# JeffWang987/MVSTER

Hardware: AMD Instinct MI355X
Metric: depth-maps/sec (DTU 512×640, 5-view, 4-stage) at 1/2/4/8 MI355X (higher is better)
Workload: dtype f32; 1 GPU; DTU mid 512x640, 5 views, 4-stage cascade 8/8/4/4 hyp, B=1 eval, 1 depth map(s) per step per GPU; launch=hipGraph replay, parallelism=replicas x1, depth_maps_in_flight_per_gpu=2

## Files before the change

### mvster_amd/csrc/conv_pers.hip

```cpp
#include "conv_args.hpp"

namespace mvconv {
namespace {


#ifdef MVSTER_TIMELINE
__device__ unsigned long long* g_ptl = nullptr;
#define MV_PTL(k)                                                                                                       \
    do {                                                                                                                \
        __builtin_amdgcn_sched_barrier(0);                                                                              \
        if (g_ptl && lane == 0 && it < 16)                                                                              \
            g_ptl[(((size_t)(blockIdx.y * gridDim.x + blockIdx.x) * 4 + wave) * 16 + it) * 8 + (k)] =                    \
                (k) < 5 ? __builtin_amdgcn_s_memtime() : (k) == 5 ? __builtin_amdgcn_s_getreg(63492)                    \
                                                         : (k) == 6 ? __builtin_amdgcn_s_getreg(63508) : tile;          \
        __builtin_amdgcn_sched_barrier(0);                                                                              \
    } while (0)
#define MV_PPTL(k, v)                                                                                                   \
    do {                                                                                                                \
        __builtin_amdgcn_sched_barrier(0);                                                                              \
        if (g_ptl && lane == 0 && hp < 16)                                                                              \
            g_ptl[(((size_t)(blockIdx.y * gridDim.x + blockIdx.x) * 8 + wave8) * 16 + hp) * 4 + (k)] = (v);           \
        __builtin_amdgcn_sched_barrier(0);                                                                              \
    } while (0)
#else
// ... 572 lines not shown
#pragma unroll
                    for (int c = 0; c < NCH; ++c) {
                        const f32x4v w = wl[(wbase + tap * NCH + c) * 64 + lane];
                        f32x4v A[MT];
#pragma unroll
                        for (int mt = 0; mt < MT; ++mt) A[mt] = patch[abase[mt] + c * 2 * PLANE + cbase + dy * RS + dx * 2];
#pragma unroll
                        for (int j = 0; j < 4; ++j)
#pragma unroll
                            for (int mt = 0; mt < MT; ++mt) acc[mt] = __builtin_amdgcn_mfma_f32_16x16x4f32(w[j], A[mt][j], acc[mt], 0, 0, 0);
                    }
                }
            wbase += kh * kw * NCH;
#pragma unroll
            for (int mt = 0; mt < MT; ++mt) {
                f32x4v v = acc[mt];
#pragma unroll
                for (int j = 0; j < 4; ++j) {
                    v[j] = fmaf(v[j], scv[j], shv[j]);
                    if (a.relu) v[j] = fmaxf(v[j], 0.0f);
                    if (SKIP) v[j] += skv[mt][j];
                }
                __builtin_amdgcn_raw_buffer_store_b128(__builtin_bit_cast(u32x4v, v), out_rsrc, ooff[mt], 0, MV_STORE_AUX);
            }
        }
        __builtin_amdgcn_s_waitcnt(0xc07f);
        __builtin_amdgcn_s_barrier();
    }
}

#ifdef MVSTER_PROBES
template <int MT, int NT, int KW, int SW, int NCH, int KD, bool WREG, int PF, bool SKIP>
__global__ void __launch_bounds__(512) conv_pp_kernel(ConvArgs a, PersArgs p) {
    using G = PersGeom<MT, KW, SW, KD>;
    constexpr int TY = G::TY, KH = G::KH, PW = G::PW, PH = G::PH, PWH = G::PWH, PLANE = G::PLANE, NBLK = G::NBLK;
    constexpr int NTAP = KD * KH * KW, TAPS2D = KH * KW;
    constexpr int BUF = NCH * 2 * PLANE;
    constexpr int NI = NCH * 2 * NBLK;
    constexpr int NIW = (NI + 3) / 4;
    constexpr int CIN = NCH * 16;
    extern __shared__ __attribute__((aligned(16))) float lds_raw[];
    const int lane = threadIdx.x & 63;
    const int wave8 = __builtin_amdgcn_readfirstlane(threadIdx.x >> 6);
    const int grp = wave8 >> 2;
    const int wave = wave8 & 3;
    f32x4v* const lds = reinterpret_cast<f32x4v*>(lds_raw) + grp * 2 * BUF;
    f32x4v* const scratch = reinterpret_cast<f32x4v*>(lds_raw) + 4 * BUF;
    f32x4v* const wl = scratch + 64;
    const int lm = lane & 15, lq = lane >> 4;
    const int nt0 = blockIdx.y * NT;
    const __amdgpu_buffer_rsrc_t in_rsrc =
        __builtin_amdgcn_make_buffer_rsrc(const_cast<float*>(a.in), (short)0, (int)a.in_bytes, 0x00020000);

    unsigned dbase[NIW];
    int dpos[NIW];
#pragma unroll
    for (int n = 0; n < NIW; ++n) {
        const int i = wave + 4 * n;
        const int c = i / (2 * NBLK), r = i - c * 2 * NBLK, pl = r / NBLK, blk = r - pl * NBLK;
        const int s = blk * 64 + lane;
        const int q1 = s & 1;
        int prow, px;
        if (SW == 1) {
            const int pix = s >> 1;
            prow = pix / PW;
            px = pix - prow * PW;
        } else {
            int t = s >> 1;
            const int xh = t % PWH;
            t /= PWH;
            prow = t >> 1;
            px = 2 * xh + (t & 1);
        }
        const bool valid = i < NI && prow < G::ROWS && px < PW;
        const int pz = KD == 1 ? 0 : prow / PH, py = prow - pz * PH;
        dpos[n] = px | (py << 8) | (pz << 16);
        dbase[n] = valid ? (unsigned)(((pz * a.Hi + py) * a.Wi + px) * (CIN * 4) + (c * 16 + pl * 8 + q1 * 4) * 4) : 0x80000000u;
    }

    auto decode_tile = [&](unsigned tile) -> TilePos {
        TilePos t;
        auto div = [&](unsigned n, int k) -> unsigned { return ((__umulhi(n, p.mul[k]) >> p.shr[k]) & ~p.one[k]) | (n & p.one[k]); };
        unsigned q = div(tile, 0);
        t.tx0 = (int)(tile - q * p.tiles_x) * 32;
        unsigned q2 = div(q, 1);
        t.ty0 = (int)(q - q2 * p.tiles_y) * TY;
        const unsigned q3 = div(q2, 2);
        t.zo = (int)(q2 - q3 * (unsigned)a.Do);
        t.b = (int)q3;
        return t;
    };

    auto dma_tile = [&](const TilePos& t, int buf, bool live) {
        const int iz0 = t.zo * a.sd - a.pd[0], iy0 = t.ty0 * SW - a.ph[0], ix0 = t.tx0 * SW - a.pw[0];
        const unsigned origin = (unsigned)((((t.b * a.Di + iz0) * a.Hi + iy0) * a.Wi + ix0) * (CIN * 4));
        const unsigned wi = live ? (unsigned)a.Wi : 0u;
        f32x4v* const dst0 = lds + buf * BUF;
#pragma unroll
        for (int n = 0; n < NIW; ++n) {
            const int i = wave + 4 * n;
            {
                const int ix = ix0 + (dpos[n] & 255), iy = iy0 + ((dpos[n] >> 8) & 255), iz = iz0 + (dpos[n] >> 16);
                bool ok = (unsigned)iy < (unsigned)a.Hi && (unsigned)ix < wi;
                if (KD > 1) ok = ok && (unsigned)iz < (unsigned)a.Di;
                const unsigned off = ok ? dbase[n] + origin : 0x80000000u;
                f32x4v* const dst = (NI % 4 == 0 || n + 1 < NIW || i < NI) ? dst0 + (i / NBLK) * PLANE + (i % NBLK) * 64 : scratch;
                __builtin_amdgcn_raw_ptr_buffer_load_lds(in_rsrc, (lds_void*)dst, 16, off, 0, 0, 0);
            }
        }
    };

    const unsigned nwg = gridDim.x;
    const unsigned first = xcd_remap(blockIdx.x, nwg);
    const unsigned ntl = first < p.ntiles ? (p.ntiles - first + nwg - 1) / nwg : 0u;
    const int kcount = (int)((ntl + 1u - (unsigned)grp) >> 1);
    auto tile_of = [&](int k) -> unsigned { return first + (unsigned)(2 * k + grp) * nwg; };
    if (kcount > 0) dma_tile(decode_tile(tile_of(0)), 0, true);
    if (grp == 0 && kcount > 1) dma_tile(decode_tile(tile_of(1)), 1, true);
    f32x4v wreg[WREG ? NTAP * NCH * NT : 1];
    const long wstep = (long)a.ntile_total * 256;
    if (WREG) {
#pragma unroll
        for (int s = 0; s < NTAP * NCH; ++s)
#pragma unroll
            for (int nt = 0; nt < NT; ++nt)
                wreg[s * NT + nt] = *reinterpret_cast<const f32x4v*>(a.wpk + s * wstep + ((long)(nt0 + nt) * 64 + lane) * 4);
    } else {
        const __amdgpu_buffer_rsrc_t w_rsrc = __builtin_amdgcn_make_buffer_rsrc(
            const_cast<float*>(a.wpk), (short)0, (int)(NTAP * NCH * wstep * 4), 0x00020000);
        for (int i = wave8; i < NTAP * NCH * NT; i += 8) {
            const int s = i / NT, nt = i - s * NT;
            const unsigned off = (unsigned)((s * wstep + (long)(nt0 + nt) * 256) * 4) + lane * 16;
            __builtin_amdgcn_raw_ptr_buffer_load_lds(w_rsrc, (lds_void*)(wl + i * 64), 16, off, 0, 0, 0);
        }
    }
    f32x4v scv[NT], shv[NT];
#pragma unroll
    for (int nt = 0; nt < NT; ++nt) {
        const int n0 = (nt0 + nt) * 16 + lq * 4;
        scv[nt] = *reinterpret_cast<const f32x4v*>(a.scale + n0);
        shv[nt] = *reinterpret_cast<const f32x4v*>(a.shift + n0);
    }
    int abase[MT];
#pragma unroll
    for (int mt = 0; mt < MT; ++mt) {
        const int t = wave * MT + mt;
        const int row = t >> 1, x = (t & 1) * 16 + lm;
        const int rs = G::ROWSLOTS;
        abase[mt] = (SW == 1 ? row * rs + x * 2 : row * 2 * rs + x * 2) + (lq >> 1) * PLANE + (lq & 1);
    }
    const __amdgpu_buffer_rsrc_t out_rsrc =
        __builtin_amdgcn_make_buffer_rsrc(a.out, (short)0, (int)p.out_bytes, 0x00020000);
    const __amdgpu_buffer_rsrc_t skip_rsrc = __builtin_amdgcn_make_buffer_rsrc(
        const_cast<float*>(SKIP ? a.skip : a.in), (short)0, SKIP ? (int)p.out_bytes : 0, 0x00020000);
    unsigned obase[MT];
    int orc[MT];
#pragma unroll
    for (int mt = 0; mt < MT; ++mt) {
        const int t = wave * MT + mt;
        const int row = t >> 1, col = (t & 1) * 16 + lm;
        orc[mt] = row | (col << 8);
        obase[mt] = (unsigned)((row * a.Wo + col) * a.cout + nt0 * 16 + lq * 4) * 4u;
    }
    auto tap_off = [&](int kz, int ky, int kx) -> int {
        const int prow = kz * PH + ky;
        return SW == 1 ? prow * G::ROWSLOTS + kx * 2 : prow * G::ROWSLOTS + (kx & 1) * PWH * 2 + (kx >> 1) * 2;
    };

    __syncthreads();

    f32x4v pacc[MT][NT], pskv[MT][NT];
    unsigned pooff[MT];
#pragma unroll
    for (int mt = 0; mt < MT; ++mt) {
        pooff[mt] = 0x80000000u;
#pragma unroll
        for (int nt = 0; nt < NT; ++nt) pacc[mt][nt] = pskv[mt][nt] = (f32x4v){0.f, 0.f, 0.f, 0.f};
    }
    auto epilogue = [&](const f32x4v (&accv)[MT][NT], const f32x4v (&skvv)[MT][NT], const unsigned (&off)[MT]) {
#pragma unroll
        for (int mt = 0; mt < MT; ++mt) {
#pragma unroll
            for (int nt = 0; nt < NT; ++nt) {
                f32x4v v = accv[mt][nt];
#pragma unroll
                for (int j = 0; j < 4; ++j) {
                    v[j] = fmaf(v[j], scv[nt][j], shv[nt][j]);
                    if (a.relu) v[j] = fmaxf(v[j], 0.0f);
                    if (SKIP) v[j] += skvv[mt][nt][j];
                }
                __builtin_amdgcn_raw_buffer_store_b128(__builtin_bit_cast(u32x4v, v), out_rsrc, off[mt] + nt * 64, 0, MV_STORE_AUX);
            }
        }
    };

    f32x4v skvN[MT][NT];
    unsigned ooffN[MT];
    TilePos here = decode_tile(kcount > 0 ? tile_of(0) : 0u);
#pragma unroll
    for (int mt = 0; mt < MT; ++mt) ooffN[mt] = 0x80000000u;
    const int nhalf = 2 * (int)((ntl + 1u) >> 1) + 1;
    {
        const unsigned oorigin = (unsigned)((((here.b * a.Do + here.zo) * a.Ho + here.ty0) * a.Wo + here.tx0) * a.cout) * 4u;
#pragma unroll
        for (int mt = 0; mt < MT; ++mt) {
            const bool ok = grp == 0 && kcount > 0 && here.ty0 + (orc[mt] & 255) < a.Ho && here.tx0 + (orc[mt] >> 8) < a.Wo;
            ooffN[mt] = ok ? obase[mt] + oorigin : 0x80000000u;
#pragma unroll
            for (int nt = 0; nt < NT; ++nt)
                skvN[mt][nt] = SKIP ? __builtin_bit_cast(f32x4v, __builtin_amdgcn_raw_buffer_load_b128(skip_rsrc, ooffN[mt] + nt * 64, 0, 0))
                                    : (f32x4v){0.f, 0.f, 0.f, 0.f};
        }
    }
    for (int hp = 0; hp < nhalf; ++hp) {
        MV_PPTL(0, __builtin_amdgcn_s_memtime());
        MV_PPTL(3, __builtin_amdgcn_s_getreg(63492));
        if ((hp & 1) == grp) {
            const int k = (hp - grp) >> 1;
            if (k < kcount) {
                const int cur = k & 1;
                f32x4v acc[MT][NT];
#pragma unroll
                for (int mt = 0; mt < MT; ++mt)
#pragma unroll
                    for (int nt = 0; nt < NT; ++nt) acc[mt][nt] = (f32x4v){0.f, 0.f, 0.f, 0.f};
                const f32x4v* patch = lds + cur * BUF;
                const int kz_lo = KD == 1 ? 0 : max(0, a.pd[0] - here.zo * a.sd), kz_hi = KD == 1 ? 1 : min(KD, a.Di + a.pd[0] - here.zo * a.sd);
#pragma unroll
                for (int kz = 0; kz < KD; ++kz) {
                    if (kz < kz_lo || kz >= kz_hi) continue;
                    f32x4v A[PF + 1][NCH][MT], Bv[PF + 1][NCH][NT];
                    auto load_tap = [&](int t2, f32x4v (&Aa)[NCH][MT], f32x4v (&Bb)[NCH][NT]) {
                        const int ky = t2 / KW, kx = t2 - ky * KW;
                        const int to = tap_off(kz, ky, kx);
                        const int tap = kz * TAPS2D + t2;
#pragma unroll
                        for (int c = 0; c < NCH; ++c) {
#pragma unroll
                            for (int mt = 0; mt < MT; ++mt) Aa[c][mt] = patch[abase[mt] + c * 2 * PLANE + to];
#pragma unroll
                            for (int nt = 0; nt < NT; ++nt)
                                Bb[c][nt] = WREG ? wreg[(tap * NCH + c) * NT + nt] : wl[((tap * NCH + c) * NT + nt) * 64 + lane];
                        }
                    };
#pragma unroll
                    for (int t2 = 0; t2 < PF && t2 < TAPS2D; ++t2) load_tap(t2, A[t2 % (PF + 1)], Bv[t2 % (PF + 1)]);
#pragma unroll
                    for (int t2 = 0; t2 < TAPS2D; ++t2) {
                        if (t2 + PF < TAPS2D) load_tap(t2 + PF, A[(t2 + PF) % (PF + 1)], Bv[(t2 + PF) % (PF + 1)]);
#pragma unroll
                        for (int c = 0; c < NCH; ++c)
#pragma unroll
                            for (int j = 0; j < 4; ++j)
#pragma unroll
                                for (int mt = 0; mt < MT; ++mt)
#pragma unroll
                                    for (int nt = 0; nt < NT; ++nt)
                                        acc[mt][nt] = __builtin_amdgcn_mfma_f32_16x16x4f32(Bv[t2 % (PF + 1)][c][nt][j], A[t2 % (PF + 1)][c][mt][j],
                                                                                           acc[mt][nt], 0, 0, 0);
                    }
                }
#pragma unroll
                for (int mt = 0; mt < MT; ++mt) {
                    pooff[mt] = ooffN[mt];
#pragma unroll
                    for (int nt = 0; nt < NT; ++nt) {
                        pacc[mt][nt] = acc[mt][nt];
                        pskv[mt][nt] = skvN[mt][nt];
                    }
                }
            }
            __builtin_amdgcn_s_waitcnt(0xc07f);
            MV_PPTL(2, k < kcount ? 1 : 0);
        } else {
            const int kn = (hp + 1 - grp) >> 1;
            epilogue(pacc, pskv, pooff);
#pragma unroll
            for (int mt = 0; mt < MT; ++mt) pooff[mt] = 0x80000000u;
            __builtin_amdgcn_sched_barrier(0);
            const bool have = kn < kcount;
            here = decode_tile(have ? tile_of(kn) : 0u);
            const unsigned oorigin = (unsigned)((((here.b * a.Do + here.zo) * a.Ho + here.ty0) * a.Wo + here.tx0) * a.cout) * 4u;
#pragma unroll
            for (int mt = 0; mt < MT; ++mt) {
                const bool ok = have && here.ty0 + (orc[mt] & 255) < a.Ho && here.tx0 + (orc[mt] >> 8) < a.Wo;
                ooffN[mt] = ok ? obase[mt] + oorigin : 0x80000000u;
#pragma unroll
                for (int nt = 0; nt < NT; ++nt)
                    skvN[mt][nt] = SKIP ? __builtin_bit_cast(f32x4v, __builtin_amdgcn_raw_buffer_load_b128(skip_rsrc, ooffN[mt] + nt * 64, 0, 0))
                                        : (f32x4v){0.f, 0.f, 0.f, 0.f};
            }
            __builtin_amdgcn_sched_barrier(0);
            const bool more = kn + 1 < kcount;
            dma_tile(decode_tile(more ? tile_of(kn + 1) : 0u), (kn + 1) & 1, more);
            MV_PPTL(2, __builtin_amdgcn_s_memtime());
            asm volatile("s_waitcnt vmcnt(%0)" ::"n"(MT * NT * (SKIP ? 2 : 1) + NIW) : "memory");
        }
        MV_PPTL(1, __builtin_amdgcn_s_memtime());
        __builtin_amdgcn_s_barrier();
    }
}
#endif

template <int NCH, int MT>
__global__ void __launch_bounds__(256) conv1x1_pers_kernel(ConvArgs a, unsigned ngroups, unsigned mtot, unsigned out_bytes) {
    constexpr int CIN = NCH * 16;
    extern __shared__ __attribute__((aligned(16))) float lds_raw[];
    f32x4v* const wl = reinterpret_cast<f32x4v*>(lds_raw);
    const int ntile = a.ntile_total;
    f32x4v* const ssl = wl + NCH * ntile * 64;
    const int lane = threadIdx.x & 63;
    const int wave = __builtin_amdgcn_readfirstlane(threadIdx.x >> 6);
    const int lm = lane & 15, lq = lane >> 4;
    const __amdgpu_buffer_rsrc_t in_rsrc =
        __builtin_amdgcn_make_buffer_rsrc(const_cast<float*>(a.in), (short)0, (int)a.in_bytes, 0x00020000);
    const __amdgpu_buffer_rsrc_t out_rsrc = __builtin_amdgcn_make_buffer_rsrc(a.out, (short)0, (int)out_bytes, 0x00020000);
    const __amdgpu_buffer_rsrc_t skip_rsrc = __builtin_amdgcn_make_buffer_rsrc(
        const_cast<float*>(a.skip_mode ? a.skip : a.in), (short)0,
        a.skip_mode == 1 ? (int)out_bytes : a.skip_mode == 2 ? (int)(out_bytes / 4) : 0, 0x00020000);
    {
        const __amdgpu_buffer_rsrc_t w_rsrc =
            __builtin_amdgcn_make_buffer_rsrc(const_cast<float*>(a.wpk), (short)0, NCH * ntile * 1024, 0x00020000);
        for (int i = wave; i < NCH * ntile; i += 4) {
            const unsigned off = (unsigned)(i * 1024 + lane * 16);
            f32x4v* const dst = wl + i * 64;
            __builtin_amdgcn_raw_ptr_buffer_load_lds(w_rsrc, (lds_void*)dst, 16, off, 0, 0, 0);
        }
        for (int i = threadIdx.x; i < ntile * 4; i += 256) {
            ssl[i] = *reinterpret_cast<const f32x4v*>(a.scale + i * 4);
            ssl[ntile * 4 + i] = *reinterpret_cast<const f32x4v*>(a.shift + i * 4);
        }
    }
    auto load_group = [&](unsigned g, f32x4v (&A)[MT][NCH], unsigned (&vox)[MT]) {
#pragma unroll
        for (int mt = 0; mt < MT; ++mt) {
            const unsigned m = ((g * 4 + wave) * MT + mt) * 16 + lm;
            vox[mt] = m;
#pragma unroll
            for (int c = 0; c < NCH; ++c) {
                const unsigned off = m < mtot ? (m * CIN + c * 16 + lq * 4) * 4u : 0x80000000u;
                A[mt][c] = __builtin_bit_cast(f32x4v, __builtin_amdgcn_raw_buffer_load_b128(in_rsrc, off, 0, 0));
            }
        }
    };
    f32x4v A[MT][NCH], An[MT][NCH];
    unsigned vox[MT], voxn[MT];
    struct Up {
        unsigned o00, o01, o10, o11;
        mv::Lerp ly, lx;
    } up[MT];
    unsigned g = blockIdx.x;
    if (g < ngroups) load_group(g, A, vox);
    __syncthreads();
    const unsigned cout4 = (unsigned)a.cout * 4u;
    for (; g < ngroups; g += gridDim.x) {
        const unsigned gn = g + gridDim.x < ngroups ? g + gridDim.x : g;
        load_group(gn, An, voxn);
        if (a.skip_mode == 2) {
            const int hh = a.HoF / 2, wh = a.WoF / 2;
#pragma unroll
            for (int mt = 0; mt < MT; ++mt) {
                const unsigned m = vox[mt] < mtot ? vox[mt] : 0u;
                const unsigned t = fast_div(m, (unsigned)a.Wo, a.div_mul[0], a.div_shr[0]);
                const int ox = (int)(m - t * (unsigned)a.Wo);
                const unsigned b = fast_div(t, (unsigned)a.Ho, a.div_mul[1], a.div_shr[1]);
                const int oy = (int)(t - b * (unsigned)a.Ho);
                up[mt].ly = mv::make_lerp(oy, hh, a.HoF);
                up[mt].lx = mv::make_lerp(ox, wh, a.WoF);
                const unsigned base = b * (unsigned)(hh * wh);
                up[mt].o00 = (base + up[mt].ly.i0 * wh + up[mt].lx.i0) * cout4;
                up[mt].o01 = (base + up[mt].ly.i0 * wh + up[mt].lx.i1) * cout4;
                up[mt].o10 = (base + up[mt].ly.i1 * wh + up[mt].lx.i0) * cout4;
                up[mt].o11 = (base + up[mt].ly.i1 * wh + up[mt].lx.i1) * cout4;
            }
        }
        f32x4v Bv[NCH];
#pragma unroll
        for (int c = 0; c < NCH; ++c) Bv[c] = wl[(c * ntile) * 64 + lane];
        for (int nt = 0; nt < ntile; ++nt) {
            f32x4v Bn[NCH];
            const int ntn = nt + 1 < ntile ? nt + 1 : nt;
#pragma unroll
            for (int c = 0; c < NCH; ++c) Bn[c] = wl[(c * ntile + ntn) * 64 + lane];
            const f32x4v sc = ssl[nt * 4 + lq], sh = ssl[ntile * 4 + nt * 4 + lq];
            f32x4v acc[MT];
#pragma unroll
            for (int mt = 0; mt < MT; ++mt) acc[mt] = (f32x4v){0.f, 0.f, 0.f, 0.f};
#pragma unroll
            for (int c = 0; c < NCH; ++c)
#pragma unroll
                for (int j = 0; j < 4; ++j)
#pragma unroll
                    for (int mt = 0; mt < MT; ++mt)
                        acc[mt] = __builtin_amdgcn_mfma_f32_16x16x4f32(Bv[c][j], A[mt][c][j], acc[mt], 0, 0, 0);
            const unsigned n0 = (unsigned)(nt * 16 + lq * 4);
#pragma unroll
            for (int mt = 0; mt < MT; ++mt) {
                const unsigned off = (n0 < (unsigned)a.cout && vox[mt] < mtot) ? vox[mt] * cout4 + n0 * 4u : 0x80000000u;
                f32x4v v = acc[mt];
#pragma unroll
                for (int j = 0; j < 4; ++j) {
                    v[j] = fmaf(v[j], sc[j], sh[j]);
                    if (a.relu) v[j] = fmaxf(v[j], 0.0f);
                }
                if (a.skip_mode == 1) {
                    const f32x4v k = __builtin_bit_cast(f32x4v, __builtin_amdgcn_raw_buffer_load_b128(skip_rsrc, off, 0, 0));
#pragma unroll
                    for (int j = 0; j < 4; ++j) v[j] += k[j];
                } else if (a.skip_mode == 2) {
                    const bool ok = n0 < (unsigned)a.cout && vox[mt] < mtot;
                    const unsigned c4 = n0 * 4u;
                    const f32x4v k00 = __builtin_bit_cast(f32x4v, __builtin_amdgcn_raw_buffer_load_b128(skip_rsrc, ok ? up[mt].o00 + c4 : 0x80000000u, 0, 0));
                    const f32x4v k01 = __builtin_bit_cast(f32x4v, __builtin_amdgcn_raw_buffer_load_b128(skip_rsrc, ok ? up[mt].o01 + c4 : 0x80000000u, 0, 0));
                    const f32x4v k10 = __builtin_bit_cast(f32x4v, __builtin_amdgcn_raw_buffer_load_b128(skip_rsrc, ok ? up[mt].o10 + c4 : 0x80000000u, 0, 0));
                    const f32x4v k11 = __builtin_bit_cast(f32x4v, __builtin_amdgcn_raw_buffer_load_b128(skip_rsrc, ok ? up[mt].o11 + c4 : 0x80000000u, 0, 0));
#pragma unroll
                    for (int j = 0; j < 4; ++j) v[j] = mv::bilerp(up[mt].ly, up[mt].lx, k00[j], k01[j], k10[j], k11[j]) + v[j];
                }
                __builtin_amdgcn_raw_buffer_store_b128(__builtin_bit_cast(u32x4v, v), out_rsrc, off, 0, MV_STORE_AUX);
            }
#pragma unroll
            for (int c = 0; c < NCH; ++c) Bv[c] = Bn[c];
        }
#pragma unroll
        for (int mt = 0; mt < MT; ++mt) {
            vox[mt] = voxn[mt];
#pragma unroll
            for (int c = 0; c < NCH; ++c) A[mt][c] = An[mt][c];
        }
    }
}


template <int MT, int NT, int KW, int SW, int NCH, int KD, bool WREG, int PF, bool SKIP, bool LD>
int launch_pers(const ConvArgs& a, int wpc, hipStream_t s) {
    using G = PersGeom<MT, KW, SW, KD>;
    constexpr int NTAP = KD * KW * KW;
    const size_t lds = (size_t)(2 * NCH * 2 * G::PLANE + 64 + (WREG ? 0 : NTAP * NCH * NT * 64)) * 16;
    if (lds > 160 * 1024) return MVSTER_ERR_UNSUPPORTED;
    auto kern = conv_pers_kernel<MT, NT, KW, SW, NCH, KD, WREG, PF, SKIP, LD>;
    static unsigned long attr_done = 0;
    if (lds > 64 * 1024 && !allow_big_lds(reinterpret_cast<const void*>(kern), attr_done)) return MVSTER_ERR_LAUNCH;
    const int g_num_cu = num_cus();
    if (g_num_cu <= 0) return MVSTER_ERR_LAUNCH;
    PersArgs p;
    if (!fill_pers_args(a, G::TY, p)) return MVSTER_ERR_UNSUPPORTED;
    const long ntiles = p.ntiles;
    p.prio = (wpc >> 4) & 1;
    wpc &= 15;
    int by_lds = (int)((160 * 1024) / lds);
    int per_cu = wpc > 0 ? wpc : (by_lds > 3 ? 3 : by_lds);
    if (per_cu > by_lds) per_cu = by_lds;
    if (per_cu < 1) per_cu = 1;
    const int ny = a.ntile_total / NT;
    long gmax = (long)g_num_cu * per_cu / ny;
    if (gmax < 1) gmax = 1;
    const long rounds = (ntiles + gmax - 1) / gmax;
    const long gx = (ntiles + rounds - 1) / rounds;
    MV_NOTE_KERNEL("conv_pers_kernel<%d, %d, %d, %d, %d, %d, %s, %d, %s, %s>", MT, NT, KW, SW, NCH, KD, WREG ? "true" : "false", PF,
                   SKIP ? "true" : "false", LD ? "true" : "false");
    hipLaunchKernelGGL(kern, dim3((unsigned)gx, ny, 1), dim3(LD ? 512 : 256), lds, s, a, p);
    return mv_check_launch();
}

template <int NCH, bool SKIP, int KS>
int launch_tpers(const ConvArgs& a, int wpc, hipStream_t s) {
    using G = PersGeom<2, KS == 5 ? 3 : 2, 1, 1>;
    const size_t lds = (size_t)(2 * NCH * 2 * G::PLANE + 64 + (KS == 5 ? 25 : 9) * NCH * 64) * 16;
    if (lds > 160 * 1024) return MVSTER_ERR_UNSUPPORTED;
    auto kern = conv_tpers_kernel<NCH, SKIP, KS>;
    static unsigned long attr_done = 0;
    if (lds > 64 * 1024 && !allow_big_lds(reinterpret_cast<const void*>(kern), attr_done)) return MVSTER_ERR_LAUNCH;
    const int ncu = num_cus();
    if (ncu <= 0) return MVSTER_ERR_LAUNCH;
    PersArgs p;
    if (!fill_pers_args(a, G::TY, p)) return MVSTER_ERR_UNSUPPORTED;
    const long ntiles = p.ntiles;
    wpc &= 15;
    const int by_lds = (int)((160 * 1024) / lds);
    int per_cu = wpc > 0 ? wpc : 2;
    if (per_cu > by_lds) per_cu = by_lds;
    if (per_cu > 2) per_cu = 2;
    long gmax = (long)ncu * per_cu / a.ntile_total;
    if (gmax < 1) gmax = 1;
    const long rounds = (ntiles + gmax - 1) / gmax;
    const long gx = (ntiles + rounds - 1) / rounds;
    MV_NOTE_KERNEL("conv_tpers_kernel<%d, %s, %d>", NCH, SKIP ? "true" : "false", KS);
    hipLaunchKernelGGL(kern, dim3((unsigned)gx, a.ntile_total, 1), dim3(512), lds, s, a, p);
    return mv_check_launch();
}

template <int KW, bool SKIP>
int launch_pers8(const ConvArgs& a, int wpc, hipStream_t s) {
    using G = PersGeom<2, KW, 2, 1>;
    const size_t lds = (size_t)(2 * G::PLANE + 64) * 16;
    auto kern = conv_pers8_kernel<KW, SKIP>;
    static unsigned long attr_done = 0;
    if (lds > 64 * 1024 && !allow_big_lds(reinterpret_cast<const void*>(kern), attr_done)) return MVSTER_ERR_LAUNCH;
    const int ncu = num_cus();
    if (ncu <= 0) return MVSTER_ERR_LAUNCH;
    PersArgs p;
    if (!fill_pers_args(a, G::TY, p)) return MVSTER_ERR_UNSUPPORTED;
    const long ntiles = p.ntiles;
    wpc &= 15;
    const int by_lds = (int)((160 * 1024) / lds);
    int per_cu = wpc > 0 ? wpc : 2;
    if (per_cu > by_lds) per_cu = by_lds;
    if (per_cu > 3) per_cu = 3;
    const long gmax = (long)ncu * per_cu;
    const long rounds = (ntiles + gmax - 1) / gmax;
    const long gx = (ntiles + rounds - 1) / rounds;
    MV_NOTE_KERNEL("conv_pers8_kernel<%d, %s>", KW, SKIP ? "true" : "false");
    hipLaunchKernelGGL(kern, dim3((unsigned)gx, 1, 1), dim3(512), lds, s, a, p);
    return mv_check_launch();
}

#ifdef MVSTER_PROBES
template <int MT, int NT, int KW, int SW, int NCH, int KD, bool WREG, int PF, bool SKIP>
int launch_pp(const ConvArgs& a, hipStream_t s) {
    using G = PersGeom<MT, KW, SW, KD>;
    constexpr int NTAP = KD * KW * KW;
    const size_t lds = (size_t)(4 * NCH * 2 * G::PLANE + 64 + (WREG ? 0 : NTAP * NCH * NT * 64)) * 16;
    if (lds > 160 * 1024) return MVSTER_ERR_UNSUPPORTED;
    auto kern = conv_pp_kernel<MT, NT, KW, SW, NCH, KD, WREG, PF, SKIP>;
    static unsigned long attr_done = 0;
    if (!allow_big_lds(reinterpret_cast<const void*>(kern), attr_done)) return MVSTER_ERR_LAUNCH;
    const int g_num_cu = num_cus();
    if (g_num_cu <= 0) return MVSTER_ERR_LAUNCH;
    PersArgs p;
    if (!fill_pers_args(a, G::TY, p)) return MVSTER_ERR_UNSUPPORTED;
    const long ntiles = p.ntiles;
    const int ny = a.ntile_total / NT;
    long gmax = (long)g_num_cu / ny;
    if (gmax < 1) gmax = 1;
    long per = (ntiles + gmax - 1) / gmax;
    if (per > 1 && (per & 1)) ++per;
    const long gx = (ntiles + per - 1) / per;
    MV_NOTE_KERNEL("conv_pp_kernel<%d, %d, %d, %d, %d, %d, %s, %d, %s>", MT, NT, KW, SW, NCH, KD, WREG ? "true" : "false", PF,
                   SKIP ? "true" : "false");
    hipLaunchKernelGGL(kern, dim3((unsigned)gx, ny, 1), dim3(512), lds, s, a, p);
    return mv_check_launch();
}
#endif

}

#ifdef MVSTER_TIMELINE
extern "C" int mvster_debug_pers_timeline(void* buf) {
    return hipMemcpyToSymbol(HIP_SYMBOL(g_ptl), &buf, sizeof(buf)) == hipSuccess ? MVSTER_OK : MVSTER_ERR_LAUNCH;
}
#endif

namespace {
template <int NCH, int MT>
int launch_1x1(const ConvArgs& a, int wpc, hipStream_t s) {
    const size_t lds = (size_t)(NCH * a.ntile_total * 64 + 2 * a.ntile_total * 4) * 16;
    const long mtot = (long)a.B * a.Do * a.Ho * a.Wo;
    const long out_bytes = mtot * a.cout * 4;
    if (lds > 160 * 1024 || a.in_bytes >= (1u << 31) || out_bytes >= (1L << 31) || a.cout % 4 != 0) return MVSTER_ERR_UNSUPPORTED;
    auto kern = conv1x1_pers_kernel<NCH, MT>;
    static unsigned long attr_done = 0;
    if (!allow_big_lds(reinterpret_cast<const void*>(kern), attr_done)) return MVSTER_ERR_LAUNCH;
    const int g_num_cu = num_cus();
    if (g_num_cu <= 0) return MVSTER_ERR_LAUNCH;
    const long ngroups = (mtot + 64 * MT - 1) / (64 * MT);
    int by_lds = (int)((160 * 1024) / lds);
    int per_cu = wpc > 0 ? wpc : 2;
    if (per_cu > by_lds) per_cu = by_lds;
    if (per_cu > 4) per_cu = 4;
    const long gmax = (long)g_num_cu * per_cu;
    const long rounds = (ngroups + gmax - 1) / gmax;
    const long gx = (ngroups + rounds - 1) / rounds;
    MV_NOTE_KERNEL("conv1x1_pers_kernel<%d, %d>", NCH, MT);
    hipLaunchKernelGGL(kern, dim3((unsigned)gx), dim3(256), lds, s, a, (unsigned)ngroups, (unsigned)mtot, (unsigned)out_bytes);
    return mv_check_launch();
}
}

int num_cus() {
    static int n = 0;
    if (n == 0) {
        int dev = 0;
        hipDeviceProp_t prop;
        if (hipGetDevice(&dev) != hipSuccess || hipGetDeviceProperties(&prop, dev) != hipSuccess) return 0;
        n = prop.multiProcessorCount;
        if (const char* e = MV_PROBE_ENV("MVSTER_CUS")) {
            const int v = atoi(e);
            if (v > 0 && v <= n) n = v;
        }
    }
    return n;
}

int dispatch_1x1(const ConvArgs& a, int mt, int wpc, hipStream_t s) {
    if (a.nclass != 1 || a.kd[0] != 1 || a.kh[0] != 1 || a.kw[0] != 1 || a.sd != 1 || a.sh != 1 || a.sw != 1 || a.osd != 1 ||
        a.osh != 1 || a.osw != 1 || a.pd[0] != 0 || a.ph[0] != 0 || a.pw[0] != 0 || a.skip_mode > 2 || a.prob_w)
        return MVSTER_ERR_UNSUPPORTED;
    if (a.skip_mode == 2 && (a.Do != 1 || (a.HoF & 1) || (a.WoF & 1))) return MVSTER_ERR_UNSUPPORTED;
    wpc &= 15;
    if (a.cin == 64 && mt == 1) return launch_1x1<4, 1>(a, wpc, s);
    if (a.cin == 64 && mt == 2) return launch_1x1<4, 2>(a, wpc, s);
    if (a.cin == 32 && mt == 1) return launch_1x1<2, 1>(a, wpc, s);
    if (a.cin == 32 && mt == 2) return launch_1x1<2, 2>(a, wpc, s);
    if (a.cin == 32 && mt == 4) return launch_1x1<2, 4>(a, wpc, s);
    if (a.cin == 16 && mt == 2) return launch_1x1<1, 2>(a, wpc, s);
    if (a.cin == 16 && mt == 4) return launch_1x1<1, 4>(a, wpc, s);
    return MVSTER_ERR_UNSUPPORTED;
}

#ifndef MVSTER_PROBES
int dispatch_pp(const ConvArgs&, int, int, hipStream_t) { return MVSTER_ERR_UNSUPPORTED; }
#else
int dispatch_pp(const ConvArgs& a, int mt, int nt, hipStream_t s) {
    if (a.nclass != 1 || a.osd != 1 || a.osh != 1 || a.osw != 1 || a.skip_mode > 1 || a.prob_w || a.cout % 16 != 0 ||
        a.sh != a.sw || a.kh[0] != a.kw[0] || a.ntile_total % nt != 0 || mt != 2 || a.cin % 16 != 0)
        return MVSTER_ERR_UNSUPPORTED;
    const int kd = a.kd[0], kw = a.kw[0], sw = a.sw, nch = a.cin / 16;
#define MV_PP(NT_, KW_, SW_, NCH_, KD_, WREG_, PF_) \
    if (nt == NT_ && kw == KW_ && sw == SW_ && nch == NCH_ && kd == KD_)                                        \
        return a.skip_mode == 1 ? launch_pp<2, NT_, KW_, SW_, NCH_, KD_, WREG_, PF_, true>(a, s)                 \
                                : launch_pp<2, NT_, KW_, SW_, NCH_, KD_, WREG_, PF_, false>(a, s);
    MV_PP(1, 3, 1, 1, 1, true, 2)
    MV_PP(2, 3, 1, 2, 1, false, 1)
    MV_PP(2, 3, 2, 1, 1, true, 1)
#undef MV_PP
    return MVSTER_ERR_UNSUPPORTED;
}
#endif

int dispatch_pers(const ConvArgs& a, int mt, int nt, int wpc, hipStream_t s) {
    if (a.nclass == 4 && a.osd == 1 && a.osh == 2 && a.osw == 2 && a.sd == 1 && a.sh == 1 && a.sw == 1 && a.skip_mode <= 1 &&
        !a.prob_w && (a.cout % 16 == 0 || a.cout == 8) && (a.cin == 16 || a.cin == 32 || a.cin == 64) && mt == 2 && nt == 1) {
        const bool k5 = a.kh[0] == 3;
        if (k5 && a.cin == 64) return MVSTER_ERR_UNSUPPORTED;
        for (int c = 0; c < 4; ++c) {
            const int py = c >> 1, px = c & 1;
            const int kh = k5 ? 3 - py : py + 1, kw = k5 ? 3 - px : px + 1, ph = k5 ? 1 - py : 0, pw = k5 ? 1 - px : 0;
            if (a.kd[c] != 1 || a.kh[c] != kh || a.kw[c] != kw || a.pd[c] || a.ph[c] != ph || a.pw[c] != pw || a.od[c] ||
                a.oh[c] != py || a.ow[c] != px || a.nsteps[c] != kh * kw * (a.cin / 16))
                return MVSTER_ERR_UNSUPPORTED;
        }
#define MV_TP(NCH_)                                                                                                   \
    return k5 ? (a.skip_mode == 1 ? launch_tpers<NCH_, true, 5>(a, wpc, s) : launch_tpers<NCH_, false, 5>(a, wpc, s)) \
              : (a.skip_mode == 1 ? launch_tpers<NCH_, true, 3>(a, wpc, s) : launch_tpers<NCH_, false, 3>(a, wpc, s));
        if (a.cin == 16) { MV_TP(1) }
        if (a.cin == 32) { MV_TP(2) }
#undef MV_TP
        return a.skip_mode == 1 ? launch_tpers<4, true, 3>(a, wpc, s) : launch_tpers<4, false, 3>(a, wpc, s);
    }
    if (a.nclass != 1 || a.osd != 1 || a.osh != 1 || a.osw != 1 || a.skip_mode > 1 || a.prob_w || a.cout % 16 != 0 ||
        a.sh != a.sw || a.kh[0] != a.kw[0] || a.ntile_total % nt != 0 || mt != 2)
        return MVSTER_ERR_UNSUPPORTED;
    const int kd = a.kd[0], kw = a.kw[0], sw = a.sw, nch = a.cin / 16;
    if (a.cin == 8 && a.cout == 16 && sw == 2 && kd == 1 && a.sd == 1 && nt == 1 && (kw == 3 || kw == 5) && a.ph[0] == kw / 2 &&
        a.pw[0] == kw / 2) {
        if (kw == 5) return a.skip_mode == 1 ? launch_pers8<5, true>(a, wpc, s) : launch_pers8<5, false>(a, wpc, s);
        return a.skip_mode == 1 ? launch_pers8<3, true>(a, wpc, s) : launch_pers8<3, false>(a, wpc, s);
    }
    if (a.cin % 16 != 0) return MVSTER_ERR_UNSUPPORTED;
#define MV_P(NT_, KW_, SW_, NCH_, KD_, WREG_, PF_) MV_Q(2, NT_, KW_, SW_, NCH_, KD_, WREG_, PF_)
    const bool ld = (wpc & 32) != 0;
#define MV_Q(MT_, NT_, KW_, SW_, NCH_, KD_, WREG_, PF_) \
    if (mt == MT_ && nt == NT_ && kw == KW_ && sw == SW_ && nch == NCH_ && kd == KD_) {                            \
        if (ld) {                                                                                                  \
              \
            if constexpr (SW_ == 2)                                                                                \
                return a.skip_mode == 1 ? launch_pers<MT_, NT_, KW_, SW_, NCH_, KD_, WREG_, PF_, true, true>(a, wpc, s)   \
                                        : launch_pers<MT_, NT_, KW_, SW_, NCH_, KD_, WREG_, PF_, false, true>(a, wpc, s); \
            return MVSTER_ERR_UNSUPPORTED;                                                                         \
        }                                                                                                          \
        return a.skip_mode == 1 ? launch_pers<MT_, NT_, KW_, SW_, NCH_, KD_, WREG_, PF_, true, false>(a, wpc, s)   \
                                : launch_pers<MT_, NT_, KW_, SW_, NCH_, KD_, WREG_, PF_, false, false>(a, wpc, s);  \
    }
    MV_P(1, 3, 1, 1, 1, true, 2)
    MV_P(2, 3, 1, 2, 1, false, 1)
    MV_P(1, 3, 1, 2, 1, false, 1)
    MV_P(1, 3, 1, 4, 1, false, 1)
    MV_P(2, 5, 2, 1, 1, false, 1)
    MV_P(1, 3, 1, 1, 3, false, 2)
    MV_P(2, 3, 2, 1, 1, false, 1)
#undef MV_P
#undef MV_Q
    return MVSTER_ERR_UNSUPPORTED;
}

}
```

Before: 1182 depth-maps/s.

## Specialize 1x1 persistent conv on tile count and skip mode with prefetch ring

Adds compile-time NTILE/SKIPM specializations of the 1x1 persistent conv kernel. The new path keeps a register ring of prefetched input groups, issues the first loads before the weight LDS fill, and issues skip loads early. It double-buffers LDS weight reads, pairs output tiles for MFMA, and picks the grid size to minimise per-CU work imbalance. The aim is to hide global-memory latency and remove runtime branching, at the cost of higher register pressure and more template instances.

```diff
diff --git a/mvster_amd/csrc/conv_pers.hip b/mvster_amd/csrc/conv_pers.hip
--- a/mvster_amd/csrc/conv_pers.hip
+++ b/mvster_amd/csrc/conv_pers.hip
@@ -898,7 +898,13 @@
 }
 #endif
 
-template <int NCH, int MT>
+#ifndef MV_1X1_PF
+#define MV_1X1_PF 1
+#endif
+#ifndef MV_1X1_PAIR
+#define MV_1X1_PAIR 1
+#endif
+template <int NCH, int MT, int NTILE, int SKIPM>
 __global__ void __launch_bounds__(256) conv1x1_pers_kernel(ConvArgs a, unsigned ngroups, unsigned mtot, unsigned out_bytes) {
     constexpr int CIN = NCH * 16;
     extern __shared__ __attribute__((aligned(16))) float lds_raw[];
@@ -914,6 +920,22 @@
     const __amdgpu_buffer_rsrc_t skip_rsrc = __builtin_amdgcn_make_buffer_rsrc(
         const_cast<float*>(a.skip_mode ? a.skip : a.in), (short)0,
         a.skip_mode == 1 ? (int)out_bytes : a.skip_mode == 2 ? (int)(out_bytes / 4) : 0, 0x00020000);
+    f32x4v R[NTILE > 0 ? MV_1X1_PF + 1 : 1][MT][NCH];
+    auto load_set = [&](unsigned gg, f32x4v (&A)[MT][NCH]) {
+#pragma unroll
+        for (int mt = 0; mt < MT; ++mt) {
+            const unsigned m = ((gg * 4 + wave) * MT + mt) * 16 + lm;
+#pragma unroll
+            for (int c = 0; c < NCH; ++c) {
+                const unsigned off = m < mtot ? (m * CIN + c * 16 + lq * 4) * 4u : 0x80000000u;
+                A[mt][c] = __builtin_bit_cast(f32x4v, __builtin_amdgcn_raw_buffer_load_b128(in_rsrc, off, 0, 0));
+            }
+        }
+    };
+    if constexpr (NTILE > 0) {
+#pragma unroll
+        for (int r = 0; r < MV_1X1_PF; ++r) load_set(blockIdx.x + r * gridDim.x, R[r]);
+    }
     {
         const __amdgpu_buffer_rsrc_t w_rsrc =
             __builtin_amdgcn_make_buffer_rsrc(const_cast<float*>(a.wpk), (short)0, NCH * ntile * 1024, 0x00020000);
@@ -926,6 +948,133 @@
             ssl[i] = *reinterpret_cast<const f32x4v*>(a.scale + i * 4);
             ssl[ntile * 4 + i] = *reinterpret_cast<const f32x4v*>(a.shift + i * 4);
         }
+    }
+    const unsigned cout4 = (unsigned)a.cout * 4u;
+    if constexpr (NTILE > 0) {
+        constexpr int RING = MV_1X1_PF + 1;
+        constexpr int NS = SKIPM == 2 ? 4 : SKIPM == 1 ? 1 : 0;
+        const unsigned stride = gridDim.x;
+        auto step = [&](unsigned gg, f32x4v (&A)[MT][NCH], f32x4v (&Anew)[MT][NCH]) {
+            unsigned obase[MT];
+            mv::Lerp ly[MT], lx[MT];
+            unsigned o00[MT], o01[MT], o10[MT], o11[MT];
+#pragma unroll
+            for (int mt = 0; mt < MT; ++mt) {
+                const unsigned m = ((gg * 4 + wave) * MT + mt) * 16 + lm;
+                obase[mt] = m < mtot ? m * cout4 : 0x80000000u;
+                if constexpr (SKIPM == 2) {
+                    const int hh = a.HoF / 2, wh = a.WoF / 2;
+                    const unsigned mm = m < mtot ? m : 0u;
+                    const unsigned t = fast_div(mm, (unsigned)a.Wo, a.div_mul[0], a.div_shr[0]);
+                    const int ox = (int)(mm - t * (unsigned)a.Wo);
+                    const unsigned b = fast_div(t, (unsigned)a.Ho, a.div_mul[1], a.div_shr[1]);
+                    const int oy = (int)(t - b * (unsigned)a.Ho);
+                    ly[mt] = mv::make_lerp(oy, hh, a.HoF);
+                    lx[mt] = mv::make_lerp(ox, wh, a.WoF);
+                    const unsigned base = b * (unsigned)(hh * wh);
+                    o00[mt] = (base + ly[mt].i0 * wh + lx[mt].i0) * cout4;
+                    o01[mt] = (base + ly[mt].i0 * wh + lx[mt].i1) * cout4;
+                    o10[mt] = (base + ly[mt].i1 * wh + lx[mt].i0) * cout4;
+                    o11[mt] = (base + ly[mt].i1 * wh + lx[mt].i1) * cout4;
+                }
+            }
+            f32x4v K[NTILE][MT][NS ? NS : 1];
+            __builtin_amdgcn_sched_barrier(0);
+#pragma unroll
+            for (int nt = 0; nt < NTILE; ++nt)
+#pragma unroll
+                for (int mt = 0; mt < MT; ++mt) {
+                    const unsigned c4 = (unsigned)(nt * 16 + lq * 4) * 4u;
+                    const bool ok = c4 < cout4 && obase[mt] != 0x80000000u;
+                    if constexpr (SKIPM == 1) {
+                        K[nt][mt][0] = __builtin_bit_cast(f32x4v, __builtin_amdgcn_raw_buffer_load_b128(skip_rsrc, ok ? obase[mt] + c4 : 0x80000000u, 0, 0));
+                    } else if constexpr (SKIPM == 2) {
+                        K[nt][mt][0] = __builtin_bit_cast(f32x4v, __builtin_amdgcn_raw_buffer_load_b128(skip_rsrc, ok ? o00[mt] + c4 : 0x80000000u, 0, 0));
+                        K[nt][mt][1] = __builtin_bit_cast(f32x4v, __builtin_amdgcn_raw_buffer_load_b128(skip_rsrc, ok ? o01[mt] + c4 : 0x80000000u, 0, 0));
+                        K[nt][mt][2] = __builtin_bit_cast(f32x4v, __builtin_amdgcn_raw_buffer_load_b128(skip_rsrc, ok ? o10[mt] + c4 : 0x80000000u, 0, 0));
+                        K[nt][mt][3] = __builtin_bit_cast(f32x4v, __builtin_amdgcn_raw_buffer_load_b128(skip_rsrc, ok ? o11[mt] + c4 : 0x80000000u, 0, 0));
+                    }
+                }
+            load_set(gg + MV_1X1_PF * stride, Anew);
+            __builtin_amdgcn_sched_barrier(0);
+            constexpr int TP = MV_1X1_PAIR ? 2 : 1;
+            f32x4v Bv[TP][NCH];
+#pragma unroll
+            for (int p = 0; p < TP; ++p)
+#pragma unroll
+                for (int c = 0; c < NCH; ++c) Bv[p][c] = wl[(c * NTILE + (p < NTILE ? p : 0)) * 64 + lane];
+#pragma unroll
+            for (int nt = 0; nt < NTILE; nt += TP) {
+                const int np = nt + TP <= NTILE ? TP : 1;
+                f32x4v Bn[TP][NCH];
+#pragma unroll
+                for (int p = 0; p < TP; ++p)
+#pragma unroll
+                    for (int c = 0; c < NCH; ++c) {
+                        const int ntn = nt + TP + p < NTILE ? nt + TP + p : nt;
+                        Bn[p][c] = wl[(c * NTILE + ntn) * 64 + lane];
+                    }
+                f32x4v acc[TP][MT];
+#pragma unroll
+                for (int p = 0; p < TP; ++p)
+#pragma unroll
+                    for (int mt = 0; mt < MT; ++mt) acc[p][mt] = (f32x4v){0.f, 0.f, 0.f, 0.f};
+#pragma unroll
+                for (int c = 0; c < NCH; ++c)
+#pragma unroll
+                    for (int j = 0; j < 4; ++j)
+#pragma unroll
+                        for (int mt = 0; mt < MT; ++mt)
+#pragma unroll
+                            for (int p = 0; p < TP; ++p)
+                                if (p < np) acc[p][mt] = __builtin_amdgcn_mfma_f32_16x16x4f32(Bv[p][c][j], A[mt][c][j], acc[p][mt], 0, 0, 0);
+                if constexpr (NS > 0) __builtin_amdgcn_sched_barrier(0);
+#pragma unroll
+                for (int mt = 0; mt < MT; ++mt)
+#pragma unroll
+                    for (int p = 0; p < TP; ++p) {
+                        if (p >= np) continue;
+                        const int t = nt + p;
+                        const f32x4v sc = ssl[t * 4 + lq], sh = ssl[NTILE * 4 + t * 4 + lq];
+                        const unsigned c4 = (unsigned)(t * 16 + lq * 4) * 4u;
+                        const unsigned off = (c4 < cout4 && obase[mt] != 0x80000000u) ? obase[mt] + c4 : 0x80000000u;
+                        f32x4v v = acc[p][mt];
+#pragma unroll
+                        for (int j = 0; j < 4; ++j) {
+                            v[j] = fmaf(v[j], sc[j], sh[j]);
+                            if (a.relu) v[j] = fmaxf(v[j], 0.0f);
+                        }
+                        if constexpr (SKIPM == 1) {
+#pragma unroll
+                            for (int j = 0; j < 4; ++j) v[j] += K[t][mt][0][j];
+                        } else if constexpr (SKIPM == 2) {
+#pragma unroll
+                            for (int j = 0; j < 4; ++j)
+                                v[j] = mv::bilerp(ly[mt], lx[mt], K[t][mt][0][j], K[t][mt][1][j], K[t][mt][2][j], K[t][mt][3][j]) + v[j];
+                        }
+                        __builtin_amdgcn_raw_buffer_store_b128(__builtin_bit_cast(u32x4v, v), out_rsrc, off, 0, MV_STORE_AUX);
+                    }
+#pragma unroll
+                for (int p = 0; p < TP; ++p)
+#pragma unroll
+                    for (int c = 0; c < NCH; ++c) Bv[p][c] = Bn[p][c];
+            }
+        };
+        unsigned g = blockIdx.x;
+        __builtin_amdgcn_s_waitcnt(0x0f70);
+        __syncthreads();
+        unsigned left = (ngroups - g + stride - 1) / stride;
+        for (; left >= (unsigned)RING; left -= RING) {
+#pragma unroll
+            for (int r = 0; r < RING; ++r) {
+                step(g, R[r], R[(r + RING - 1) % RING]);
+                g += stride;
+            }
+        }
+#pragma unroll
+        for (int r = 0; r < RING - 1; ++r)
+            if ((unsigned)r < left) step(g + r * stride, R[r], R[(r + RING - 1) % RING]);
+        return;
     }
     auto load_group = [&](unsigned g, f32x4v (&A)[MT][NCH], unsigned (&vox)[MT]) {
 #pragma unroll
@@ -948,7 +1097,6 @@
     unsigned g = blockIdx.x;
     if (g < ngroups) load_group(g, A, vox);
     __syncthreads();
-    const unsigned cout4 = (unsigned)a.cout * 4u;
     for (; g < ngroups; g += gridDim.x) {
         const unsigned gn = g + gridDim.x < ngroups ? g + gridDim.x : g;
         load_group(gn, An, voxn);
@@ -1148,13 +1296,13 @@
 #endif
 
 namespace {
-template <int NCH, int MT>
+template <int NCH, int MT, int NTILE, int SKIPM>
 int launch_1x1(const ConvArgs& a, int wpc, hipStream_t s) {
     const size_t lds = (size_t)(NCH * a.ntile_total * 64 + 2 * a.ntile_total * 4) * 16;
     const long mtot = (long)a.B * a.Do * a.Ho * a.Wo;
     const long out_bytes = mtot * a.cout * 4;
     if (lds > 160 * 1024 || a.in_bytes >= (1u << 31) || out_bytes >= (1L << 31) || a.cout % 4 != 0) return MVSTER_ERR_UNSUPPORTED;
-    auto kern = conv1x1_pers_kernel<NCH, MT>;
+    auto kern = conv1x1_pers_kernel<NCH, MT, NTILE, SKIPM>;
     static unsigned long attr_done = 0;
     if (!allow_big_lds(reinterpret_cast<const void*>(kern), attr_done)) return MVSTER_ERR_LAUNCH;
     const int g_num_cu = num_cus();
@@ -1164,10 +1312,21 @@
     int per_cu = wpc > 0 ? wpc : 2;
     if (per_cu > by_lds) per_cu = by_lds;
     if (per_cu > 4) per_cu = 4;
-    const long gmax = (long)g_num_cu * per_cu;
+    long gmax = (long)g_num_cu * per_cu;
+    if (NTILE > 0) {
+        long best = 0;
+        for (int k = 1; k <= per_cu; ++k) {
+            const long slots = (long)g_num_cu * k;
+            const long share = k * ((ngroups + slots - 1) / slots);
+            if (k == 1 || share < best) {
+                best = share;
+                gmax = slots;
+            }
+        }
+    }
     const long rounds = (ngroups + gmax - 1) / gmax;
     const long gx = (ngroups + rounds - 1) / rounds;
-    MV_NOTE_KERNEL("conv1x1_pers_kernel<%d, %d>", NCH, MT);
+    MV_NOTE_KERNEL("conv1x1_pers_kernel<%d, %d, %d, %d>", NCH, MT, NTILE, SKIPM);
     hipLaunchKernelGGL(kern, dim3((unsigned)gx), dim3(256), lds, s, a, (unsigned)ngroups, (unsigned)mtot, (unsigned)out_bytes);
     return mv_check_launch();
 }
@@ -1194,13 +1353,24 @@
         return MVSTER_ERR_UNSUPPORTED;
     if (a.skip_mode == 2 && (a.Do != 1 || (a.HoF & 1) || (a.WoF & 1))) return MVSTER_ERR_UNSUPPORTED;
     wpc &= 15;
-    if (a.cin == 64 && mt == 1) return launch_1x1<4, 1>(a, wpc, s);
-    if (a.cin == 64 && mt == 2) return launch_1x1<4, 2>(a, wpc, s);
-    if (a.cin == 32 && mt == 1) return launch_1x1<2, 1>(a, wpc, s);
-    if (a.cin == 32 && mt == 2) return launch_1x1<2, 2>(a, wpc, s);
-    if (a.cin == 32 && mt == 4) return launch_1x1<2, 4>(a, wpc, s);
-    if (a.cin == 16 && mt == 2) return launch_1x1<1, 2>(a, wpc, s);
-    if (a.cin == 16 && mt == 4) return launch_1x1<1, 4>(a, wpc, s);
+    const int nt = a.ntile_total, sm = a.skip_mode;
+#define MV_1X1_FIXED(NCH_, NTILE_, SKIPM_)                                            \
+    if (a.cin == NCH_ * 16 && nt == NTILE_ && sm == SKIPM_ && (mt == 1 || mt == 2))  \
+        return mt == 1 ? launch_1x1<NCH_, 1, NTILE_, SKIPM_>(a, wpc, s) : launch_1x1<NCH_, 2, NTILE_, SKIPM_>(a, wpc, s);
+    MV_1X1_FIXED(4, 9, 0)
+    MV_1X1_FIXED(4, 5, 0)
+    MV_1X1_FIXED(4, 4, 0)
+    MV_1X1_FIXED(4, 4, 1)
+    MV_1X1_FIXED(2, 4, 2)
+#undef MV_1X1_FIXED
+    if (a.cin == 64 && mt == 1) return launch_1x1<4, 1, 0, -1>(a, wpc, s);
+    if (a.cin == 64 && mt == 2) return launch_1x1<4, 2, 0, -1>(a, wpc, s);
+    if (a.cin == 32 && mt == 1) return launch_1x1<2, 1, 0, -1>(a, wpc, s);
+    if (a.cin == 32 && mt == 2) return launch_1x1<2, 2, 0, -1>(a, wpc, s);
+    if (a.cin == 32 && mt == 4) return launch_1x1<2, 4, 0, -1>(a, wpc, s);
+    if (a.cin == 16 && mt == 1) return launch_1x1<1, 1, 0, -1>(a, wpc, s);
+    if (a.cin == 16 && mt == 2) return launch_1x1<1, 2, 0, -1>(a, wpc, s);
+    if (a.cin == 16 && mt == 4) return launch_1x1<1, 4, 0, -1>(a, wpc, s);
     return MVSTER_ERR_UNSUPPORTED;
 }
 
```

Result: no change. 1180 depth-maps/s (-0.2%).
